# ElijahHyndman/PAPTeam_OpticalFlow

Measured on AMD Instinct MI355X. Metric: Mpix/s per frame-pair (fixed SOR iters) at 1920x1080; max-abs d(u,v) vs ref, higher is better.
Workload: dtype f64

## Files before the change

papteam_opticalflow_amd/csrc/sor.hip:

```cpp
#include <algorithm>
#include <cstdio>
#include <cstdlib>
#include <cstring>
#include <type_traits>

#include "common.h"

namespace papof {

namespace {

#ifndef PAPOF_V_DM6
#define PAPOF_V_DM6 4
#endif
#ifndef PAPOF_V_DM8
#define PAPOF_V_DM8 5
#endif
#ifndef PAPOF_V_FDM6
#define PAPOF_V_FDM6 3
#endif
#ifndef PAPOF_V_FDM8
#define PAPOF_V_FDM8 4
#endif
#ifndef PAPOF_V_FMIDPOLL
#define PAPOF_V_FMIDPOLL 10
#endif
#ifndef PAPOF_V_FSELECTIVE
#define PAPOF_V_FSELECTIVE false
#endif
#ifndef PAPOF_V_MIDPOLL
#define PAPOF_V_MIDPOLL 8
#endif
#ifndef PAPOF_V_SLEEP
#define PAPOF_V_SLEEP 1
#endif
constexpr int kProgStride = 32;
constexpr unsigned kSpinLimit = 4u << 20;

struct ExactArgs {
    const double *phi, *xy, *a1, *a2, *b1, *b2;
    double *du, *dv;
    unsigned* prog;
    unsigned* abort;
    int H, W, nb, ns, hp, npos, qt, rt, npos_d, n_sor;
    int xcd_affine;
    int k0;
    int b0, nbl;
    double nalpha, om1;
    unsigned long long* dbg;
    unsigned long long* stamp;
    double* peer_du;
    unsigned* peer_prog;
    int top_cut;
    int bot_cut;
    size_t bs_coef, bs_d, bs_prog;
    int skip_dead;
};

__device__ __forceinline__ void stamp_now(unsigned long long* s) {
    if (s && (blockIdx.x | threadIdx.x) == 0u) *s = __builtin_amdgcn_s_memrealtime();
}

__device__ __forceinline__ double ld_agent(const double* p) {
    return __hip_atomic_load(p, __ATOMIC_RELAXED, __HIP_MEMORY_SCOPE_AGENT);
}
__device__ __forceinline__ void st_agent(double* p, double v) {
    __hip_atomic_store(p, v, __ATOMIC_RELAXED, __HIP_MEMORY_SCOPE_AGENT);
}

template <bool DPP>
__device__ __forceinline__ double from_above(double x) {
    if (DPP) {
        int lo = __builtin_amdgcn_update_dpp(0, __double2loint(x), 0x138, 0xf, 0xf, true);
        int hi = __builtin_amdgcn_update_dpp(0, __double2hiint(x), 0x138, 0xf, 0xf, true);
        return __hiloint2double(hi, lo);
    }
    return __shfl_up(x, 1);
}
template <bool DPP>
__device__ __forceinline__ double from_below(double x) {
    if (DPP) {
        int lo = __builtin_amdgcn_update_dpp(0, __double2loint(x), 0x130, 0xf, 0xf, true);
        int hi = __builtin_amdgcn_update_dpp(0, __double2hiint(x), 0x130, 0xf, 0xf, true);
        return __hiloint2double(hi, lo);
    }
    return __shfl_down(x, 1);
}

__global__ void k_xlane_probe(int* out) {
    const int lane = threadIdx.x;
    const double v = (double)(lane + 1);
    out[lane] = (int)from_above<true>(v);
    out[64 + lane] = (int)from_below<true>(v);
}

typedef unsigned u32x4 __attribute__((ext_vector_type(4)));
struct D2 {
    double x, y;
};
__device__ __forceinline__ D2 as_d2(u32x4 v) {
    D2 r;
    __builtin_memcpy(&r, &v, sizeof r);
    return r;
}
__device__ __forceinline__ u32x4 as_u4(double x, double y) {
    D2 d{x, y};
    u32x4 r;
    __builtin_memcpy(&r, &d, sizeof r);
    return r;
}
constexpr int kAuxPlain = 0, kAuxSc1 = 16;
constexpr unsigned kOob = 0x80000000u;
constexpr unsigned kBlock = kLanes * 16u;

template <int T0, int T1, class F, class... Args>
__device__ __forceinline__ void static_for(F&& f, Args... args) {
    if constexpr (T0 < T1) {
        static_for<T0, T1 - 1>(f, args...);
        f(std::integral_constant<int, T1 - 1>{}, args...);
    }
}
template <int N, class F>
__device__ __forceinline__ void static_for(F&& f) {
    static_for<0, N>(f);
}

__device__ __forceinline__ D2 sor_cell(double wl, double duL, double dvL, double wu, double duU, double dvU, double wc,
                                       double duR, double dvR, double duD, double dvD, double nalpha, double xy,
                                       double duC, double dvC, double om1, double a1, double a2, double b1, double b2) {
    double s1 = wl * duL, s2 = wl * dvL;
    s1 += wc * duR;
    s2 += wc * dvR;
    s1 += wu * duU;
    s2 += wu * dvU;
    s1 += wc * duD;
    s2 += wc * dvD;
    s1 *= nalpha;
    s2 *= nalpha;
    s1 += xy * dvC;
    const double duN = om1 * duC + a1 * (b1 - s1);
    s2 += xy * duN;
    const double dvN = om1 * dvC + a2 * (b2 - s2);
    return D2{duN, dvN};
}

template <int R>
struct Slots {
    u32x4 pa[R], pb[R], pc[R];
    u32x4 pd[R];
};

struct Task {
    __amdgpu_buffer_rsrc_t ra, rb, rc, rd;
    __amdgpu_buffer_rsrc_t rp;
    __amdgpu_buffer_rsrc_t rd2, rp2;
};

__device__ __forceinline__ void publish(const Task& T, unsigned lane_off, unsigned steps) {
    __builtin_amdgcn_raw_buffer_store_b32(steps, T.rp, lane_off, 0, 16 );
}

struct BufAt {
    unsigned lane, uniform;
};
struct LaneOffs {
    unsigned pa;
    unsigned pbc;
    unsigned pd;
    unsigned st;
    unsigned pos_c;
    unsigned pos_d;
    unsigned hs;
    __device__ __forceinline__ BufAt unknowns_at(int s) const { return BufAt{pd, (unsigned)s * pos_d}; }
};

template <int R, int t, class Lane>
__device__ __forceinline__ void load_coef(const Task& T, const Lane& L, int s, Slots<R>& c) {
    const unsigned off = (unsigned)s * L.pos_c;
    c.pa[t] = __builtin_amdgcn_raw_buffer_load_b128(T.ra, L.pa, off, kAuxPlain);
    c.pb[t] = __builtin_amdgcn_raw_buffer_load_b128(T.rb, L.pbc, off, kAuxPlain);
    c.pc[t] = __builtin_amdgcn_raw_buffer_load_b128(T.rc, L.pbc, off, kAuxPlain);
}
template <int R, int t, class Lane>
__device__ __forceinline__ void load_unknowns(const Task& T, const Lane& L, int s, Slots<R>& c) {
    const BufAt at = L.unknowns_at(s);
    c.pd[t] = __builtin_amdgcn_raw_buffer_load_b128(T.rd, at.lane, at.uniform, kAuxSc1);
}
template <int R, int t, class Lane>
__device__ __forceinline__ void load_slot(const Task& T, const Lane& L, int s, Slots<R>& c) {
    load_coef<R, t>(T, L, s, c);
    load_unknowns<R, t>(T, L, s, c);
}
template <int R, class Lane>
__device__ __forceinline__ void fill_coef(const Task& T, const Lane& L, Slots<R>& c) {
    static_for<R>([&](auto t) __attribute__((always_inline)) { load_coef<R, t()>(T, L, t(), c); });
}
template <int R, class Lane>
__device__ __forceinline__ void fill_unknowns(const Task& T, const Lane& L, Slots<R>& c) {
    static_for<R>([&](auto t) __attribute__((always_inline)) { load_unknowns<R, t()>(T, L, t(), c); });
}

struct State {
    double duL, dvL, phiL, duC, dvC;
};

template <bool DPP>
__device__ __forceinline__ D2 wave_cell(const State& S, double om1, double nalpha, const D2& pa, const D2& pb,
                                        const D2& pc, double duR, double dvR) {
    const double duD = from_below<DPP>(duR);
    const double dvD = from_below<DPP>(dvR);
    const double leftU = S.phiL * S.duL;
    const double leftV = S.phiL * S.dvL;
    const double upU = from_above<DPP>(leftU);
    const double upV = from_above<DPP>(leftV);
    return sor_cell(1.0, leftU, leftV, 1.0, upU, upV, pa.x, duR, dvR, duD, dvD, nalpha, pa.y, S.duC, S.dvC, om1, pb.x, pb.y,
                    pc.x, pc.y);
}

__device__ __forceinline__ void store_data_guard() { asm volatile("s_nop 1" ::: "memory"); }

__device__ __forceinline__ double moved(double x) {
    double y;
    asm volatile("v_mov_b64 %0, %1" : "=v"(y) : "v"(x));
    return y;
}

template <int R, int t, bool DPP, bool SPLIT = false>
__device__ __forceinline__ void step(const ExactArgs& A, const Task& T, const LaneOffs& L, double om1, int s,
                                     Slots<R>& c, State& S) {
    const D2 pa = as_d2(c.pa[t]), pb = as_d2(c.pb[t]), pc = as_d2(c.pc[t]), pd = as_d2(c.pd[t]);
    const double phiC = pa.x, duR = pd.x, dvR = pd.y;
    const D2 n = wave_cell<DPP>(S, om1, A.nalpha, pa, pb, pc, duR, dvR);
    __builtin_amdgcn_raw_buffer_store_b128(as_u4(n.x, n.y), T.rd, L.st, (unsigned)s * L.pos_d, kAuxSc1);
    if (SPLIT)
        __builtin_amdgcn_raw_buffer_store_b128(as_u4(n.x, n.y), T.rd2, L.hs, (unsigned)s * L.pos_d, kAuxSc1);
    store_data_guard();
    S.duL = n.x;
    S.dvL = n.y;
    S.phiL = moved(phiC);
    S.duC = moved(duR);
    S.dvC = moved(dvR);
    asm volatile("" ::: "memory");
    load_slot<R, t>(T, L, s + R, c);
}

struct Polls {
    unsigned own, up, dn2;
};
struct Deps {
    unsigned *own, *up, *dn2;
    bool has_own, has_up, has_dn2;
};
__device__ __forceinline__ Polls poll(const Deps& d) {
    Polls p;
    p.own = d.has_own ? __hip_atomic_load(d.own, __ATOMIC_RELAXED, __HIP_MEMORY_SCOPE_AGENT) : 0x7fffffffu;
    p.up = d.has_up ? __hip_atomic_load(d.up, __ATOMIC_RELAXED, __HIP_MEMORY_SCOPE_AGENT) : 0x7fffffffu;
    p.dn2 = d.has_dn2 ? __hip_atomic_load(d.dn2, __ATOMIC_RELAXED, __HIP_MEMORY_SCOPE_AGENT) : 0x7fffffffu;
    return p;
}
__device__ __forceinline__ unsigned uni(unsigned v) { return (unsigned)__builtin_amdgcn_readfirstlane((int)v); }
__device__ __forceinline__ Polls uni(const Polls& p) { return Polls{uni(p.own), uni(p.up), uni(p.dn2)}; }

template <int OWN, int UP>
__device__ __forceinline__ bool covered(const Polls& p, int ns, int s_end) {
    return p.own >= (unsigned)min(ns, s_end + OWN) && p.up >= (unsigned)min(ns, s_end + UP) &&
           p.dn2 >= (unsigned)min(ns, max(0, s_end - 62));
}

__device__ __forceinline__ void end_task() { __builtin_amdgcn_endpgm(); }

template <int OWN, int UP, bool SELECTIVE = false>
__device__ __forceinline__ bool wait_covered(const ExactArgs& A, const Polls& pl, const Deps& d, int s_end) {
    Polls p = uni(pl);
    if (!covered<OWN, UP>(p, A.ns, s_end)) {
        unsigned spins = 0;
        do {
            __builtin_amdgcn_s_sleep(PAPOF_V_SLEEP);
            if ((++spins & 255u) == 0u) {
                if (uni(__hip_atomic_load(A.abort, __ATOMIC_RELAXED, __HIP_MEMORY_SCOPE_AGENT)) != 0u) return false;
                if (spins > kSpinLimit) {
                    __hip_atomic_store(A.abort, 1u, __ATOMIC_RELAXED, __HIP_MEMORY_SCOPE_AGENT);
                    return false;
                }
            }
            if (!SELECTIVE) {
                p = uni(poll(d));
                continue;
            }
            const unsigned need_own = (unsigned)min(A.ns, s_end + OWN), need_up = (unsigned)min(A.ns, s_end + UP);
            const unsigned need_dn2 = (unsigned)min(A.ns, max(0, s_end - 62));
            if (p.own < need_own) p.own = uni(__hip_atomic_load(d.own, __ATOMIC_RELAXED, __HIP_MEMORY_SCOPE_AGENT));
            if (p.up < need_up) p.up = uni(__hip_atomic_load(d.up, __ATOMIC_RELAXED, __HIP_MEMORY_SCOPE_AGENT));
            if (p.dn2 < need_dn2) p.dn2 = uni(__hip_atomic_load(d.dn2, __ATOMIC_RELAXED, __HIP_MEMORY_SCOPE_AGENT));
        } while (!covered<OWN, UP>(p, A.ns, s_end));
    }
    __builtin_amdgcn_fence(__ATOMIC_ACQUIRE, "wavefront");
    return true;
}

__device__ __forceinline__ bool task_of_block(const ExactArgs& A, int& u, int& b) {
    if (A.xcd_affine) {
        const int nf = A.nb >> 3, rem = A.nb & 7, S = 8 * nf + (rem ? 8 : 0);
        const int ul = blockIdx.x / S;
        u = A.k0 + ul;
        const int r = blockIdx.x - ul * S;
        if (r < 8 * nf) {
            b = r;
        } else {
            const int j = r - 8 * nf - (nf ? u % (9 - rem) : 0);
            b = 8 * nf + j;
            if (j < 0 || j >= rem) return false;
        }
    } else {
        const int ul = blockIdx.x / A.nbl;
        u = A.k0 + ul;
        b = A.b0 + (blockIdx.x - ul * A.nbl);
    }
    return true;
}

__device__ __forceinline__ unsigned plane_descriptors(const ExactArgs& A, Task& T) {
    const unsigned plane_bytes = (unsigned)(((size_t)A.npos * A.hp + kLanes) * 16u);
    const unsigned par_bytes = (unsigned)A.npos_d * (unsigned)A.nb * kBlock;
    T.ra = __builtin_amdgcn_make_buffer_rsrc((void*)A.phi, 0, plane_bytes, 0x00020000);
    T.rb = __builtin_amdgcn_make_buffer_rsrc((void*)A.a1, 0, plane_bytes, 0x00020000);
    T.rc = __builtin_amdgcn_make_buffer_rsrc((void*)A.b1, 0, plane_bytes, 0x00020000);
    T.rd = __builtin_amdgcn_make_buffer_rsrc((void*)A.du, 0, 2u * par_bytes, 0x00020000);
    return par_bytes;
}

struct Pipe {
    Polls pl;
    unsigned ma, mb;
};
template <int R, int DM, bool MIDPOLL, int OWN, int UP, bool SELECTIVE, class Run, class Publish>
__device__ __forceinline__ void pipeline_iteration(const ExactArgs& A, const Deps& D, const State& S, Pipe& P, int i,
                                                   bool first, Run&& run, Publish&& publish) {
    constexpr int H = R / 2;
    constexpr int CA = H + DM - R, CB = DM;
    static_assert(CA >= 0 && CA < H && CB >= H && CB < R, "marker consumption points");
    if (!wait_covered<OWN, UP, SELECTIVE>(A, P.pl, D, (i + 2) * R)) end_task();
    Polls pn{0u, 0u, 0u};
    if (!MIDPOLL) pn = poll(D);
    static_for<0, CA>(run, i * R);
    if (!first) {
        asm volatile("" ::"v"(P.ma), "v"(S.duL), "v"(S.dvL) : "memory");
        if (uni(P.ma) != 0u) end_task();
        publish((unsigned)min(A.ns, (i - 1) * R + H));
    }
    static_for<CA, H>(run, i * R);
    P.ma = __hip_atomic_load(A.abort, __ATOMIC_RELAXED, __HIP_MEMORY_SCOPE_AGENT);
    if (MIDPOLL) pn = poll(D);
    static_for<H, CB>(run, i * R);
    if (!first) {
        asm volatile("" ::"v"(P.mb), "v"(S.duL), "v"(S.dvL) : "memory");
        if (uni(P.mb) != 0u) end_task();
        publish((unsigned)min(A.ns, i * R));
    }
    static_for<CB, R>(run, i * R);
    P.mb = __hip_atomic_load(A.abort, __ATOMIC_RELAXED, __HIP_MEMORY_SCOPE_AGENT);
    P.pl = pn;
}

template <int R, bool DPP, bool SPLIT = false>
__global__ __launch_bounds__(64) void k_sor_exact(ExactArgs A_in) {
    static_assert(R >= 4 && R % 2 == 0, "two markers per iteration");
    ExactArgs A = A_in;
    {
        const size_t p = blockIdx.y;
        A.phi += p * A.bs_coef;
        A.a1 += p * A.bs_coef;
        A.b1 += p * A.bs_coef;
        A.du += p * A.bs_d;
        A.prog += p * A.bs_prog;
    }
    stamp_now(A.stamp);
    const unsigned lane = threadIdx.x;
    int k, b;
    if (!task_of_block(A, k, b)) return;
    const int ns = A.ns;
    const bool ghost = lane == 0 || lane == kLanes - 1;
    unsigned long long* const dbg = A.dbg ? A.dbg + (size_t)(k * A.nb + b) * 8 : nullptr;
    if (dbg) dbg[0] = __builtin_amdgcn_s_memrealtime();
    Task T;
    const unsigned par_bytes = plane_descriptors(A, T);
    const int r0 = kBandRows * b - k - 1;
    LaneOffs L;
    L.pos_c = (unsigned)A.hp * 16u;
    L.pos_d = (unsigned)A.nb * kBlock;
    const unsigned base = ((unsigned)(r0 + A.qt) * (unsigned)A.hp + (unsigned)(r0 + A.rt) + lane) * 16u;
    const int row = r0 + (int)lane;
    const bool dead = !SPLIT && A.skip_dead != 0 && (row < 0 || row >= A.H);
    L.pa = dead ? kOob : base;
    L.pbc = (ghost || dead) ? kOob : base;
    const unsigned mine = (unsigned)(k & 1) * par_bytes, prev = (unsigned)((k + 1) & 1) * par_bytes;
    L.st = dead ? kOob : mine + L.pos_d + (unsigned)b * kBlock + lane * 16u;
    const bool cut_top = SPLIT && A.top_cut && b == A.b0, cut_bot = SPLIT && A.bot_cut && b == A.b0 + A.nbl - 1;
    const unsigned up_cell = cut_top ? (unsigned)(k >> 1) : 62u;
    const unsigned pd_above = b > 0 ? mine + 64u * L.pos_d + (unsigned)(b - 1) * kBlock + up_cell * 16u : kOob;
    L.hs = (cut_bot && lane == kLanes - 2) ? mine + L.pos_d + (unsigned)b * kBlock + (unsigned)(k >> 1) * 16u : kOob;
    T.rd2 = __builtin_amdgcn_make_buffer_rsrc((void*)((SPLIT && A.peer_du) ? A.peer_du : A.du), 0, 2u * par_bytes, 0x00020000);
    L.pd = dead ? kOob : (lane == 0 ? pd_above : (k > 0 ? prev + L.pos_d + (unsigned)b * kBlock + (lane - 1u) * 16u : kOob));
    const double om1 = ghost ? 1.0 : A.om1;

    const unsigned prog_bytes = (unsigned)A.n_sor * (unsigned)A.nb * kProgStride * 4u;
    T.rp = __builtin_amdgcn_make_buffer_rsrc((void*)A.prog, 0, prog_bytes, 0x00020000);
    T.rp2 = __builtin_amdgcn_make_buffer_rsrc((void*)((SPLIT && A.peer_prog) ? A.peer_prog : A.prog), 0, prog_bytes, 0x00020000);
    const unsigned my_prog = lane == 0 ? (unsigned)(k * A.nb + b) * kProgStride * 4u : kOob;
    const unsigned my_prog2 = cut_bot ? my_prog : kOob;
    Deps D;
    D.has_own = k > 0;
    D.has_up = b > 0;
    D.has_dn2 = k > 1 && b + 1 < A.nb && !cut_bot;
    D.own = A.prog + ((size_t)(k - 1) * A.nb + b) * kProgStride;
    D.up = A.prog + ((size_t)k * A.nb + (b - 1)) * kProgStride;
    D.dn2 = A.prog + ((size_t)(k - 2) * A.nb + (b + 1)) * kProgStride;
    const auto publish_all = [&](unsigned steps) {
        publish(T, my_prog, steps);
        if (SPLIT) __builtin_amdgcn_raw_buffer_store_b32(steps, T.rp2, my_prog2, 0, 16 );
    };

    const int n_iter = (ns + R - 1) / R;
    State S;
    S.duL = S.dvL = S.phiL = 0.0;
    Slots<R> c;

    fill_coef(T, L, c);
    Pipe P{poll(D), 0u, 0u};
    if (!wait_covered<0, 63, true>(A, P.pl, D, R)) end_task();
    {
        const unsigned first = (lane != 0 || L.pd == kOob) ? kOob : L.pd - L.pos_d;
        const D2 c0 = as_d2(__builtin_amdgcn_raw_buffer_load_b128(T.rd, first, 0, kAuxSc1));
        S.duC = c0.x;
        S.dvC = c0.y;
    }
    if (dbg) dbg[1] = __builtin_amdgcn_s_memrealtime();
    fill_unknowns(T, L, c);
    P.pl = poll(D);

    constexpr int DM = R >= 10 ? R - 3 : (R == 8 ? PAPOF_V_DM8 : (R == 6 ? PAPOF_V_DM6 : R / 2));
    const auto iteration = [&](int i, bool first) {
        pipeline_iteration<R, DM, R >= PAPOF_V_MIDPOLL, 0, 63, true>(
            A, D, S, P, i, first,
            [&](auto t, int s0) __attribute__((always_inline)) { step<R, t(), DPP, SPLIT>(A, T, L, om1, s0 + t(), c, S); },
            publish_all);
    };
    iteration(0, true);
    if (dbg) dbg[2] = __builtin_amdgcn_s_memrealtime();
    for (int i = 1; i < n_iter; ++i) {
        iteration(i, false);
        if (dbg && i < 4) dbg[2 + i] = __builtin_amdgcn_s_memrealtime();
    }
    asm volatile("s_waitcnt vmcnt(0)" ::: "memory");
    publish_all((unsigned)ns);
    if (dbg) dbg[6] = __builtin_amdgcn_s_memrealtime();
}

struct FLane {
    unsigned m1;
    double om1a;
    double om1b;
    bool first_out;
    bool own_block;
};

template <int R, int t, bool DPP, bool SKIP2, bool ID2>
__device__ __forceinline__ void f_step(const ExactArgs& A, const Task& T, const LaneOffs& L, const FLane& F, int s,
                                       Slots<R>& c, State& S1, State& S2) {
    const double nalpha = A.nalpha;
    constexpr int t2 = (t + R - 2) % R;
    const double duR2 = S1.duL, dvR2 = S1.dvL;
    double duN2, dvN2;
    if (SKIP2) {
        duN2 = 0.0;
        dvN2 = 0.0;
    } else {
        const D2 qa = as_d2(c.pa[t2]), qc = as_d2(c.pc[t2]);
        const u32x4 qbm = ID2 ? (c.pb[t2] & u32x4{0u, 0u, 0u, 0u}) : c.pb[t2];
        const D2 qb = as_d2(qbm);
        const D2 n2 = wave_cell<DPP>(S2, F.om1b, nalpha, qa, qb, qc, duR2, dvR2);
        duN2 = n2.x;
        dvN2 = n2.y;
        S2.phiL = moved(qa.x);
    }
    const D2 pa = as_d2(c.pa[t]), pc = as_d2(c.pc[t]), pd = as_d2(c.pd[t]);
    const u32x4 pbm = c.pb[t] & u32x4{F.m1, F.m1, F.m1, F.m1};
    const D2 pb = as_d2(pbm);
    const double phiC = pa.x, duR = pd.x, dvR = pd.y;
    const D2 n1 = wave_cell<DPP>(S1, F.om1a, nalpha, pa, pb, pc, duR, dvR);
    const double duN = n1.x, dvN = n1.y;
    const double o1 = F.first_out ? duN : duN2, o2 = F.first_out ? dvN : dvN2;
    __builtin_amdgcn_raw_buffer_store_b128(as_u4(o1, o2), T.rd, L.st, (unsigned)s * L.pos_d, kAuxSc1);
    store_data_guard();
    S2.duL = duN2;
    S2.dvL = dvN2;
    S2.duC = duR2;
    S2.dvC = dvR2;
    S1.duL = duN;
    S1.dvL = dvN;
    S1.phiL = phiC;
    S1.duC = moved(duR);
    S1.dvC = moved(dvR);
    asm volatile("" ::: "memory");
    load_unknowns<R, t>(T, L, s + R, c);
    if (!SKIP2) load_coef<R, t2>(T, L, s - 2 + R, c);
}

template <int R, bool DPP, bool ID2>
__device__ __forceinline__ void f_run(const ExactArgs& A, const Task& T, const LaneOffs& L, const FLane& F,
                                      const Deps& D, unsigned my_prog) {
    const int ns = A.ns;
    const int n_iter = (ns + R - 1) / R;
    State S1, S2;
    S1.duL = S1.dvL = S1.phiL = 0.0;
    S2.duL = S2.dvL = S2.phiL = S2.duC = S2.dvC = 0.0;
    Slots<R> c;
    fill_coef(T, L, c);
    Pipe P{poll(D), 0u, 0u};
    if (!wait_covered<1, 64, PAPOF_V_FSELECTIVE>(A, P.pl, D, R)) end_task();
    {
        const unsigned first = (F.own_block || L.pd == kOob) ? kOob : L.pd - L.pos_d;
        const D2 c0 = as_d2(__builtin_amdgcn_raw_buffer_load_b128(T.rd, first, 0, kAuxSc1));
        S1.duC = c0.x;
        S1.dvC = c0.y;
    }
    fill_unknowns(T, L, c);
    P.pl = poll(D);
    constexpr int DM = R == 6 ? PAPOF_V_FDM6 : (R == 8 ? PAPOF_V_FDM8 : R - 3);
    const auto iteration = [&](int i, auto first) {
        pipeline_iteration<R, DM, R >= PAPOF_V_FMIDPOLL, 1, 64, PAPOF_V_FSELECTIVE>(
            A, D, S1, P, i, first(),
            [&](auto t, int s0) __attribute__((always_inline)) {
                f_step<R, t(), DPP, first() && t() < 2, ID2>(A, T, L, F, s0 + t(), c, S1, S2);
            },
            [&](unsigned steps) __attribute__((always_inline)) { publish(T, my_prog, steps); });
    };
    iteration(0, std::true_type{});
    for (int i = 1; i < n_iter; ++i) iteration(i, std::false_type{});
    asm volatile("s_waitcnt vmcnt(0)" ::: "memory");
    publish(T, my_prog, (unsigned)ns);
}

template <int R, bool DPP>
__global__ __launch_bounds__(64) void k_sor_fused(ExactArgs A) {
    static_assert(R >= 6 && R % 2 == 0, "two markers per iteration; coefficient slots live two extra steps");
    stamp_now(A.stamp);
    const unsigned lane = threadIdx.x;
    const int pairs = (A.n_sor + 1) >> 1;
    int q, b;
    if (!task_of_block(A, q, b)) return;
    Task T;
    const unsigned par_bytes = plane_descriptors(A, T);
    const int r0 = kFusedRows * b - 2 * q - 2;
    LaneOffs L;
    L.pos_c = (unsigned)A.hp * 16u;
    L.pos_d = (unsigned)A.nb * kBlock;
    const unsigned base = ((unsigned)(r0 + A.qt) * (unsigned)A.hp + (unsigned)(r0 + A.rt) + lane) * 16u;
    L.pa = base;
    L.pbc = (lane == 0 || lane == kLanes - 1) ? kOob : base;
    const unsigned mine = (unsigned)(q & 1) * par_bytes, prev = (unsigned)((q + 1) & 1) * par_bytes;
    L.st = lane == kLanes - 1 ? kOob : mine + L.pos_d + (unsigned)b * kBlock + lane * 16u;
    const unsigned pd1 = b > 0 ? mine + 63u * L.pos_d + (unsigned)(b - 1) * kBlock + 62u * 16u : kOob;
    const unsigned pd0 = b > 0 ? mine + 65u * L.pos_d + (unsigned)(b - 1) * kBlock + 61u * 16u : kOob;
    const unsigned pd_own = q > 0 ? prev + 2u * L.pos_d + (unsigned)b * kBlock + (lane - 2u) * 16u : kOob;
    L.pd = lane == 0 ? pd0 : (lane == 1 ? pd1 : pd_own);
    FLane F;
    const bool real1 = lane >= 2 && lane <= kLanes - 2;
    F.m1 = real1 ? 0xffffffffu : 0u;
    F.om1a = real1 ? A.om1 : 1.0;
    F.om1b = (lane == 0 || lane == kLanes - 1) ? 1.0 : A.om1;
    if ((A.n_sor & 1) && q == pairs - 1) F.om1b = 1.0;
    F.first_out = lane == kLanes - 2;
    F.own_block = lane >= 2;

    const unsigned prog_bytes = (unsigned)A.n_sor * (unsigned)A.nb * kProgStride * 4u;
    T.rp = __builtin_amdgcn_make_buffer_rsrc((void*)A.prog, 0, prog_bytes, 0x00020000);
    const unsigned my_prog = lane == 0 ? (unsigned)(q * A.nb + b) * kProgStride * 4u : kOob;
    Deps D;
    D.has_own = q > 0;
    D.has_up = b > 0;
    D.has_dn2 = q > 1 && b + 1 < A.nb;
    D.own = A.prog + ((size_t)(q - 1) * A.nb + b) * kProgStride;
    D.up = A.prog + ((size_t)q * A.nb + (b - 1)) * kProgStride;
    D.dn2 = A.prog + ((size_t)(q - 2) * A.nb + (b + 1)) * kProgStride;
    if ((A.n_sor & 1) && q == pairs - 1)
        f_run<R, DPP, true>(A, T, L, F, D, my_prog);
    else
        f_run<R, DPP, false>(A, T, L, F, D, my_prog);
}

struct GroupArgs {
    const double *phi, *a1, *b1;
    double* du;
    unsigned* prog;
    unsigned* abort;
    int nb, ns, hp, npos, qt, rt, npos_d, n_sor;
    int xcd_affine;
    int g0;
    unsigned long long* dbg;
    unsigned halo_off;
    double nalpha, om1;
    unsigned long long* stamp;
};

constexpr int kRing = 16;

struct GLane {
    unsigned pa, pbc;
    unsigned pd, pd_step;
    unsigned st;
    unsigned hs;
    unsigned pos_c, pos_d;
    __device__ __forceinline__ BufAt unknowns_at(int s) const { return BufAt{pd + (unsigned)s * pd_step, 0u}; }
};

typedef __attribute__((address_space(3))) u32x4 lds_u32x4;
typedef __attribute__((address_space(3))) volatile unsigned lds_word;

template <int R, int t, bool DPP, bool FROM_LDS, bool TO_LDS>
__device__ __forceinline__ void g_step(const GroupArgs& A, const Task& T, const GLane& L, lds_u32x4* ring_out,
                                       unsigned lane, double om1, int s, Slots<R>& c, const u32x4 (&lpd)[R / 2],
                                       State& S) {
    const D2 pa = as_d2(c.pa[t]), pb = as_d2(c.pb[t]), pc = as_d2(c.pc[t]);
    u32x4 raw = c.pd[t];
    if (FROM_LDS) {
        const u32x4 l = lpd[t % (R / 2)];
        raw = lane != 0 ? l : raw;
    }
    const D2 pd = as_d2(raw);
    const double phiC = pa.x, duR = pd.x, dvR = pd.y;
    const D2 n = wave_cell<DPP>(S, om1, A.nalpha, pa, pb, pc, duR, dvR);
    const u32x4 out = as_u4(n.x, n.y);
    if (TO_LDS)
        ring_out[(s & (kRing - 1)) * kLanes + lane] = out;
    else
        __builtin_amdgcn_raw_buffer_store_b128(out, T.rd, L.st, (unsigned)s * L.pos_d, kAuxSc1);
    __builtin_amdgcn_raw_buffer_store_b128(out, T.rd, L.hs + (unsigned)s * 16u, 0, kAuxSc1);
    store_data_guard();
    S.duL = n.x;
    S.dvL = n.y;
    S.phiL = moved(phiC);
    S.duC = moved(duR);
    S.dvC = moved(dvR);
    asm volatile("" ::: "memory");
    load_slot<R, t>(T, L, s + R, c);
}

template <int R, int T0, int T1, bool DPP, bool FROM_LDS, bool TO_LDS>
__device__ __forceinline__ void g_steps(const GroupArgs& A, const Task& T, const GLane& L, lds_u32x4* ring_out,
                                        unsigned lane, double om1, int s0, Slots<R>& c, const u32x4 (&lpd)[R / 2],
                                        State& S) {
    static_for<T0, T1>([&](auto t) __attribute__((always_inline)) {
        g_step<R, t(), DPP, FROM_LDS, TO_LDS>(A, T, L, ring_out, lane, om1, s0 + t(), c, lpd, S);
    });
}

__device__ __forceinline__ void lds_store_lane0(lds_word* p, unsigned v) {
    unsigned long long saved;
    asm volatile("s_mov_b64 %0, exec\n\ts_mov_b64 exec, 1\n\tds_write_b32 %1, %2\n\ts_mov_b64 exec, %0"
                 : "=&s"(saved)
                 : "v"((unsigned)(unsigned long long)(const volatile void __attribute__((address_space(3)))*)p), "v"(v)
                 : "memory");
}
__device__ __forceinline__ bool lds_wait_ge(lds_word* p, unsigned need, lds_word* group_abort) {
    unsigned spins = 0;
    while (uni(*p) < need) {
        __builtin_amdgcn_s_sleep(1);
        if ((++spins & 255u) == 0u && (uni(*group_abort) != 0u || spins > (kSpinLimit << 3))) return false;
    }
    asm volatile("" ::: "memory");
    return true;
}

struct GWaveCtx {
    lds_u32x4 *ring_in, *ring_out;
    lds_word *done_in, *taken_in, *done_out, *taken_out;
    lds_word* group_abort;
    int task;
    unsigned my_prog;
    Deps D;
    int ns, n_iter;
};

template <int R, bool DPP, bool FROM_LDS, bool TO_LDS>
__device__ __forceinline__ void g_run_wave(const GroupArgs& A, const Task& T, const GLane& L, const GWaveCtx& W,
                                           unsigned lane, double om1) {
    constexpr int H = R / 2;
    const int ns = W.ns;
    ExactArgs X;
    X.abort = A.abort;
    X.ns = ns;
    const auto give_up = [&]() {
        lds_store_lane0(W.group_abort, 1u);
        __hip_atomic_store(A.abort, 1u, __ATOMIC_RELAXED, __HIP_MEMORY_SCOPE_AGENT);
    };
    State S;
    S.duL = S.dvL = S.phiL = 0.0;
    Slots<R> c;
    u32x4 lpd[H];
#pragma unroll
    for (int q = 0; q < H; q++) lpd[q] = u32x4{0u, 0u, 0u, 0u};
    const unsigned lcell = lane > 0 ? lane - 1u : 0u;

    unsigned long long t_cov = 0, t_in = 0, t_out = 0, t_start = 0;
    const bool dbg = A.dbg != nullptr;
    fill_coef(T, L, c);
    Polls pl = poll(W.D);
    if (!wait_covered<1, 63>(X, pl, W.D, 2 * R)) return give_up();
    if (dbg) t_start = __builtin_amdgcn_s_memtime();
    {
        const unsigned first = L.pd == kOob ? kOob : L.pd - L.pd_step;
        const D2 c0 = as_d2(__builtin_amdgcn_raw_buffer_load_b128(T.rd, first, 0, kAuxSc1));
        S.duC = c0.x;
        S.dvC = c0.y;
    }
    fill_unknowns(T, L, c);

    const auto half_begin = [&](int sa) -> bool {
        if (FROM_LDS) {
            const unsigned long long ta = dbg ? __builtin_amdgcn_s_memtime() : 0;
            if (!lds_wait_ge(W.done_in, (unsigned)(sa + H), W.group_abort)) return false;
            if (dbg) t_in += __builtin_amdgcn_s_memtime() - ta;
#pragma unroll
            for (int q = 0; q < H; q++) lpd[q] = W.ring_in[((sa + q) & (kRing - 1)) * kLanes + lcell];
        }
        const unsigned long long tb = dbg ? __builtin_amdgcn_s_memtime() : 0;
        if (TO_LDS && sa + H > kRing && !lds_wait_ge(W.taken_out, (unsigned)(sa + H - kRing), W.group_abort))
            return false;
        if (dbg) t_out += __builtin_amdgcn_s_memtime() - tb;
        return true;
    };
    const auto half_end = [&](int sa) {
        if (FROM_LDS) {
            asm volatile("" ::: "memory");
            lds_store_lane0(W.taken_in, (unsigned)(sa + H));
        }
        if (TO_LDS) {
            asm volatile("s_waitcnt lgkmcnt(0)" ::: "memory");
            lds_store_lane0(W.done_out, (unsigned)(sa + H));
        }
    };

    constexpr int DL = R - 3, CA = H + DL - R, CB = DL;
    static_assert(CA >= 0 && CA < H && CB >= H && CB < R, "marker consumption points");
    unsigned ma = 0u, mb = 0u;
    const auto iteration = [&](int i, bool first) -> bool {
        const unsigned long long tc = dbg ? __builtin_amdgcn_s_memtime() : 0;
        if (!first && !wait_covered<1, 63>(X, pl, W.D, (i + 2) * R)) return false;
        if (dbg) t_cov += __builtin_amdgcn_s_memtime() - tc;
        const Polls pn = poll(W.D);
        const int s0 = i * R;
        if (!half_begin(s0)) return false;
        g_steps<R, 0, CA, DPP, FROM_LDS, TO_LDS>(A, T, L, W.ring_out, lane, om1, s0, c, lpd, S);
        if (!first) {
            asm volatile("" ::"v"(ma), "v"(S.duL), "v"(S.dvL) : "memory");
            if (uni(ma) != 0u) return false;
            publish(T, W.my_prog, (unsigned)min(ns, s0 - R + H));
        }
        g_steps<R, CA, H, DPP, FROM_LDS, TO_LDS>(A, T, L, W.ring_out, lane, om1, s0, c, lpd, S);
        ma = __hip_atomic_load(A.abort, __ATOMIC_RELAXED, __HIP_MEMORY_SCOPE_AGENT);
        half_end(s0);
        if (!half_begin(s0 + H)) return false;
        g_steps<R, H, CB, DPP, FROM_LDS, TO_LDS>(A, T, L, W.ring_out, lane, om1, s0, c, lpd, S);
        if (!first) {
            asm volatile("" ::"v"(mb), "v"(S.duL), "v"(S.dvL) : "memory");
            if (uni(mb) != 0u) return false;
            publish(T, W.my_prog, (unsigned)min(ns, s0));
        }
        g_steps<R, CB, R, DPP, FROM_LDS, TO_LDS>(A, T, L, W.ring_out, lane, om1, s0, c, lpd, S);
        mb = __hip_atomic_load(A.abort, __ATOMIC_RELAXED, __HIP_MEMORY_SCOPE_AGENT);
        half_end(s0 + H);
        pl = pn;
        return true;
    };
    if (!iteration(0, true)) return give_up();
    for (int i = 1; i < W.n_iter; ++i)
        if (!iteration(i, false)) return give_up();
    asm volatile("s_waitcnt vmcnt(0)" ::: "memory");
    publish(T, W.my_prog, (unsigned)ns);
    if (dbg) {
        unsigned long long* o = A.dbg + (size_t)W.task * 4;
        o[0] = __builtin_amdgcn_s_memtime() - t_start;
        o[1] = t_cov;
        o[2] = t_in;
        o[3] = t_out;
    }
}

template <int R, int M, bool DPP>
__global__ __launch_bounds__(64 * M) void k_sor_group(GroupArgs A) {
    static_assert(R >= 6 && R % 2 == 0 && R <= kRing, "half-iterations of R/2 steps; the ring holds two of them");
    __shared__ u32x4 ring[(M > 1 ? M - 1 : 1) * kRing * kLanes];
    __shared__ unsigned lds_done[M];
    __shared__ unsigned lds_taken[M];
    __shared__ unsigned lds_abort;
    stamp_now(A.stamp);
    const unsigned lane = threadIdx.x & 63u;
    const int m = __builtin_amdgcn_readfirstlane((int)(threadIdx.x >> 6));
    lds_store_lane0((lds_word*)&lds_done[m], 0u);
    lds_store_lane0((lds_word*)&lds_taken[m], 0u);
    lds_store_lane0((lds_word*)&lds_abort, 0u);
    __syncthreads();
    int g, b;
    if (A.xcd_affine) {
        const int x = blockIdx.x & 7, y = blockIdx.x >> 3, nb8 = (A.nb + 7) >> 3;
        const int gl = y / nb8;
        g = A.g0 + gl;
        b = (y - gl * nb8) * 8 + x;
        if (b >= A.nb) return;
    } else {
        const int gl = blockIdx.x / A.nb;
        g = A.g0 + gl;
        b = blockIdx.x - gl * A.nb;
    }
    const int k = g * M + m;
    if (k >= A.n_sor) return;
    const bool ghost = lane == 0 || lane == kLanes - 1;
    const bool from_lds = m > 0, to_planes = m == M - 1 || k == A.n_sor - 1;
    GWaveCtx W;
    lds_u32x4* const ring3 = (lds_u32x4*)ring;
    W.ring_in = ring3 + (m > 0 ? m - 1 : 0) * kRing * kLanes;
    W.ring_out = ring3 + (m < M - 1 ? m : 0) * kRing * kLanes;
    W.done_in = (lds_word*)&lds_done[m > 0 ? m - 1 : 0];
    W.taken_in = (lds_word*)&lds_taken[m > 0 ? m - 1 : 0];
    W.done_out = (lds_word*)&lds_done[m];
    W.taken_out = (lds_word*)&lds_taken[m];
    W.group_abort = (lds_word*)&lds_abort;
    W.task = k * A.nb + b;
    W.ns = A.ns;
    W.n_iter = (A.ns + R - 1) / R;

    Task T;
    const unsigned plane_bytes = (unsigned)(((size_t)A.npos * A.hp + kLanes) * 16u);
    const unsigned par_bytes = (unsigned)A.npos_d * (unsigned)A.nb * kBlock;
    const unsigned all_bytes = A.halo_off + (unsigned)A.n_sor * (unsigned)A.nb * (unsigned)A.npos_d * 16u;
    T.ra = __builtin_amdgcn_make_buffer_rsrc((void*)A.phi, 0, plane_bytes, 0x00020000);
    T.rb = __builtin_amdgcn_make_buffer_rsrc((void*)A.a1, 0, plane_bytes, 0x00020000);
    T.rc = __builtin_amdgcn_make_buffer_rsrc((void*)A.b1, 0, plane_bytes, 0x00020000);
    T.rd = __builtin_amdgcn_make_buffer_rsrc((void*)A.du, 0, all_bytes, 0x00020000);
    const int r0 = kBandRows * b - k - 1;
    GLane L;
    L.pos_c = (unsigned)A.hp * 16u;
    L.pos_d = (unsigned)A.nb * kBlock;
    const unsigned base = ((unsigned)(r0 + A.qt) * (unsigned)A.hp + (unsigned)(r0 + A.rt) + lane) * 16u;
    L.pa = base;
    L.pbc = ghost ? kOob : base;
    const unsigned mine = (unsigned)(g & 1) * par_bytes, prev = (unsigned)((g + 1) & 1) * par_bytes;
    L.st = to_planes ? mine + L.pos_d + (unsigned)b * kBlock + lane * 16u : kOob;
    const auto halo_row = [&](int kk, int bb) {
        return A.halo_off + (unsigned)((kk * A.nb + bb) * A.npos_d) * 16u;
    };
    const unsigned pd_halo = b > 0 ? halo_row(k, b - 1) + 64u * 16u : kOob;
    const unsigned pd_plane = prev + L.pos_d + (unsigned)b * kBlock + (lane - 1u) * 16u;
    L.pd = lane == 0 ? pd_halo : (from_lds ? kOob : pd_plane);
    L.pd_step = lane == 0 ? 16u : (from_lds ? 0u : L.pos_d);
    L.hs = (lane == kLanes - 2 && b + 1 < A.nb) ? halo_row(k, b) + 16u : kOob;
    const double om1 = ghost ? 1.0 : A.om1;

    T.rp = __builtin_amdgcn_make_buffer_rsrc((void*)A.prog, 0, (unsigned)A.n_sor * (unsigned)A.nb * kProgStride * 4u, 0x00020000);
    W.my_prog = lane == 0 ? (unsigned)(k * A.nb + b) * kProgStride * 4u : kOob;
    W.D.has_own = m == 0 && k > 0;
    W.D.has_up = b > 0;
    W.D.has_dn2 = false;
    W.D.own = A.prog + ((size_t)(k - 1) * A.nb + b) * kProgStride;
    W.D.up = A.prog + ((size_t)k * A.nb + (b - 1)) * kProgStride;
    W.D.dn2 = W.D.own;
    if (from_lds) {
        if (to_planes)
            g_run_wave<R, DPP, true, false>(A, T, L, W, lane, om1);
        else
            g_run_wave<R, DPP, true, true>(A, T, L, W, lane, om1);
    } else {
        if (to_planes)
            g_run_wave<R, DPP, false, false>(A, T, L, W, lane, om1);
        else
            g_run_wave<R, DPP, false, true>(A, T, L, W, lane, om1);
    }
}

typedef double f64x2 __attribute__((ext_vector_type(2)));

struct BlockedArgs {
    const double *phi, *xy, *a1, *a2, *b1, *b2;
    const double *su, *sv;
    double *du, *dv;
    int H, W;
    Rect out;
    int g;
    int hs0;
    int cw, ch, ntx, nblk;
    int shift;
    unsigned long long* stamp;
    double nalpha, om1;
};

template <bool VEC>
__device__ __forceinline__ f64x2 load_pair(const double* __restrict__ plane, size_t o, bool ok0, bool ok1) {
    f64x2 r = {0.0, 0.0};
    if (VEC) {
        if (ok0) r = *reinterpret_cast<const f64x2*>(plane + o);
    } else {
        if (ok0) r.x = plane[o];
        if (ok1) r.y = plane[o + 1];
    }
    return r;
}

template <int MODE, int NW, int RPT, bool VEC>
__global__ __launch_bounds__(NW * 64) void k_sor_blocked(BlockedArgs A) {
    constexpr int RH = NW * RPT, S = kLanes + 1, CELLS = (RH + 2) * S + 2;
    __shared__ f64x2 lds[2][CELLS];
    stamp_now(A.stamp);
    const int t = threadIdx.x & 63;
    const int w = __builtin_amdgcn_readfirstlane((int)(threadIdx.x >> 6));
    const int per = (A.nblk + 7) >> 3;
    const int tile = (int)(blockIdx.x & 7u) * per + (int)(blockIdx.x >> 3);
    if ((int)(blockIdx.x >> 3) >= per || tile >= A.nblk) return;
    const int by = tile / A.ntx, bx = tile - by * A.ntx;
    const int cx0 = A.out.x0 + bx * A.cw, cx1 = min(cx0 + A.cw, A.out.x1);
    const int cy0 = A.out.y0 + by * A.ch, cy1 = min(cy0 + A.ch, A.out.y1);
    const int rx0 = max(0, cx0 - A.g - A.shift), rx1 = min(A.W, cx1 + A.g);
    const int ry0 = max(0, cy0 - A.g), ry1 = min(A.H, cy1 + A.g);
    const int W = A.W;
    const int j0 = rx0 + 2 * t;
    const int r0 = w * RPT;
    const int q0 = (ry0 + rx0 + r0) & 1;

    double ph[RPT][3], up[2], cxy[RPT][2], ca1[RPT][2], ca2[RPT][2], cb1[RPT][2], cb2[RPT][2];
    f64x2 u0[RPT], v0[RPT];
    {
        const int iu = ry0 + r0 - 1;
        const bool rok = iu >= 0 && iu < ry1;
        const f64x2 pu = load_pair<VEC>(A.phi, (size_t)max(iu, 0) * W + j0, rok && j0 < rx1, rok && j0 + 1 < rx1);
        up[0] = pu.x;
        up[1] = pu.y;
    }
    static_for<RPT>([&](auto RR) __attribute__((always_inline)) {
        constexpr int rr = decltype(RR)::value;
        const int i = ry0 + r0 + rr;
        const bool rok = i < ry1, ok0 = rok && j0 < rx1, ok1 = rok && j0 + 1 < rx1;
        const size_t o = (size_t)min(i, A.H - 1) * W + j0;
        const f64x2 p = load_pair<VEC>(A.phi, o, ok0, ok1);
        const f64x2 x = load_pair<VEC>(A.xy, o, ok0, ok1);
        const f64x2 q1 = load_pair<VEC>(A.a1, o, ok0, ok1);
        const f64x2 q2 = load_pair<VEC>(A.a2, o, ok0, ok1);
        const f64x2 e1 = load_pair<VEC>(A.b1, o, ok0, ok1);
        const f64x2 e2 = load_pair<VEC>(A.b2, o, ok0, ok1);
        u0[rr] = f64x2{0.0, 0.0};
        v0[rr] = f64x2{0.0, 0.0};
        if (A.su) {
            u0[rr] = load_pair<VEC>(A.su, o, ok0, ok1);
            v0[rr] = load_pair<VEC>(A.sv, o, ok0, ok1);
        }
        ph[rr][1] = p.x;
        ph[rr][2] = p.y;
        cxy[rr][0] = x.x;
        cxy[rr][1] = x.y;
        ca1[rr][0] = q1.x;
        ca1[rr][1] = q1.y;
        ca2[rr][0] = q2.x;
        ca2[rr][1] = q2.y;
        cb1[rr][0] = e1.x;
        cb1[rr][1] = e1.y;
        cb2[rr][0] = e2.x;
        cb2[rr][1] = e2.y;
    });
    static_for<RPT>([&](auto RR) __attribute__((always_inline)) {
        constexpr int rr = decltype(RR)::value;
        const double left = __shfl_up(ph[rr][2], 1);
        ph[rr][0] = t == 0 ? 0.0 : left;
    });

    const int idx0 = (r0 + 1) * S + t + 1;
    static_for<RPT>([&](auto RR) __attribute__((always_inline)) {
        constexpr int rr = decltype(RR)::value;
        const int c0 = (q0 + rr) & 1;
        lds[c0][idx0 + rr * S] = f64x2{u0[rr].x, v0[rr].x};
        lds[c0 ^ 1][idx0 + rr * S] = f64x2{u0[rr].y, v0[rr].y};
        if (t == 0) {
            lds[0][idx0 + rr * S - 1] = f64x2{0.0, 0.0};
            lds[1][idx0 + rr * S - 1] = f64x2{0.0, 0.0};
        }
    });
    if (w == 0) {
        lds[0][t] = f64x2{0.0, 0.0};
        lds[1][t] = f64x2{0.0, 0.0};
        if (t == 0) {
            lds[0][S - 1] = f64x2{0.0, 0.0};
            lds[1][S - 1] = f64x2{0.0, 0.0};
        }
    }
    if (w == NW - 1) {
        lds[0][(RH + 1) * S + t] = f64x2{0.0, 0.0};
        lds[1][(RH + 1) * S + t] = f64x2{0.0, 0.0};
        if (t < 3) {
            lds[0][(RH + 1) * S + 64 + t - 1 + 1] = f64x2{0.0, 0.0};
            lds[1][(RH + 1) * S + 64 + t - 1 + 1] = f64x2{0.0, 0.0};
        }
    }
    __syncthreads();

    const int ox0 = rx0 > 0, ox1 = rx1 < A.W, oy0 = ry0 > 0, oy1 = ry1 < A.H;
    const int rw = rx1 - rx0, rh = ry1 - ry0;
    const double nalpha = A.nalpha, om1 = A.om1;
    const auto cell = [&](auto RR, auto PP, int cc) __attribute__((always_inline)) -> f64x2 {
        constexpr int rr = decltype(RR)::value, p = decltype(PP)::value;
        const int idx = idx0 + rr * S;
        const f64x2* __restrict__ Lo = lds[cc ^ 1];
        const f64x2 own = lds[cc][idx];
        const f64x2 L = Lo[idx - 1 + p], R = Lo[idx + p], U = Lo[idx - S], D = Lo[idx + S];
        const double pc = ph[rr][1 + p], wl = ph[rr][p];
        double wu;
        if constexpr (rr > 0)
            wu = ph[rr - 1][1 + p];
        else
            wu = up[p];
        const D2 n = sor_cell(wl, L.x, L.y, wu, U.x, U.y, pc, R.x, R.y, D.x, D.y, nalpha, cxy[rr][p], own.x,
                              own.y, om1, ca1[rr][p], ca2[rr][p], cb1[rr][p], cb2[rr][p]);
        return f64x2{n.x, n.y};
    };
    if (MODE == PAPOF_SOR_REDBLACK) {
        const auto half = [&](auto PARC, int m, int c) __attribute__((always_inline)) {
            constexpr int PAR = decltype(PARC)::value;
            const int fx0 = ox0 * (m + 1), fx1 = rw - ox1 * (m + 1), fy0 = oy0 * (m + 1), fy1 = rh - oy1 * (m + 1);
            if (r0 + RPT <= fy0 || r0 >= fy1) {
                __syncthreads();
                return;
            }
            if constexpr (NW < 16) {
                constexpr int IL = NW == 12 ? 2 : RPT;
                static_assert(RPT % IL == 0, "row groups");
                static_for<RPT / IL>([&](auto GG) __attribute__((always_inline)) {
                    constexpr int g0 = decltype(GG)::value * IL;
                    f64x2 nw[IL];
                    static_for<IL>([&](auto QQ) __attribute__((always_inline)) {
                        constexpr int rr = g0 + decltype(QQ)::value;
                        nw[decltype(QQ)::value] = cell(std::integral_constant<int, rr>{}, std::integral_constant<int, (PAR + rr) & 1>{}, c);
                    });
                    static_for<IL>([&](auto QQ) __attribute__((always_inline)) {
                        constexpr int rr = g0 + decltype(QQ)::value;
                        constexpr int p = (PAR + rr) & 1;
                        const int r = r0 + rr, lc = 2 * t + p;
                        if (r >= fy0 && r < fy1 && lc >= fx0 && lc < fx1) lds[c][idx0 + rr * S] = nw[decltype(QQ)::value];
                    });
                });
            } else {
                static_for<RPT>([&](auto RR) __attribute__((always_inline)) {
                    constexpr int rr = decltype(RR)::value;
                    constexpr int p = (PAR + rr) & 1;
                    const int r = r0 + rr;
                    if (r >= fy0 && r < fy1) {
// ... 880 lines not shown
```

Before: 213.8.

## Shorten unknowns prefetch lead by one step and split phi from a/b loads

Changes the software pipeline in the wavefront SOR kernels so the unknowns (du,dv) and phi slots are refilled one step later (R-1 ahead) while a/b coefficients stay R ahead. The dependency wait thresholds drop by one step, so waves can start an iteration sooner after upstream progress. It also removes the explicit v_mov_b64 register copies by tying the store-data hazard guard to the stored values. The risk is less latency hiding for the unknown loads and subtle slot-indexing or hazard mistakes.

```diff
diff --git a/papteam_opticalflow_amd/csrc/sor.hip b/papteam_opticalflow_amd/csrc/sor.hip
--- a/papteam_opticalflow_amd/csrc/sor.hip
+++ b/papteam_opticalflow_amd/csrc/sor.hip
@@ -171,13 +171,21 @@
     unsigned pos_c;
     unsigned pos_d;
     unsigned hs;
-    __device__ __forceinline__ BufAt unknowns_at(int s) const { return BufAt{pd, (unsigned)s * pos_d}; }
+    int pd_lead = 0;
+    __device__ __forceinline__ void lead_unknowns(int steps) {
+        pd = pd == kOob ? kOob : pd + (unsigned)steps * pos_d;
+        pd_lead = steps;
+    }
+    __device__ __forceinline__ BufAt unknowns_at(int s) const { return BufAt{pd, (unsigned)(s - pd_lead) * pos_d}; }
 };
 
 template <int R, int t, class Lane>
-__device__ __forceinline__ void load_coef(const Task& T, const Lane& L, int s, Slots<R>& c) {
+__device__ __forceinline__ void load_phi(const Task& T, const Lane& L, int s, Slots<R>& c) {
+    c.pa[t] = __builtin_amdgcn_raw_buffer_load_b128(T.ra, L.pa, (unsigned)s * L.pos_c, kAuxPlain);
+}
+template <int R, int t, class Lane>
+__device__ __forceinline__ void load_ab(const Task& T, const Lane& L, int s, Slots<R>& c) {
     const unsigned off = (unsigned)s * L.pos_c;
-    c.pa[t] = __builtin_amdgcn_raw_buffer_load_b128(T.ra, L.pa, off, kAuxPlain);
     c.pb[t] = __builtin_amdgcn_raw_buffer_load_b128(T.rb, L.pbc, off, kAuxPlain);
     c.pc[t] = __builtin_amdgcn_raw_buffer_load_b128(T.rc, L.pbc, off, kAuxPlain);
 }
@@ -187,17 +195,26 @@
     c.pd[t] = __builtin_amdgcn_raw_buffer_load_b128(T.rd, at.lane, at.uniform, kAuxSc1);
 }
 template <int R, int t, class Lane>
-__device__ __forceinline__ void load_slot(const Task& T, const Lane& L, int s, Slots<R>& c) {
-    load_coef<R, t>(T, L, s, c);
-    load_unknowns<R, t>(T, L, s, c);
-}
-template <int R, class Lane>
+__device__ __forceinline__ void refill(const Task& T, const Lane& L, int s, Slots<R>& c) {
+    constexpr int tp = (t + R - 1) % R;
+    load_phi<R, tp>(T, L, s + R - 1, c);
+    load_ab<R, t>(T, L, s + R, c);
+    load_unknowns<R, tp>(T, L, s + R - 1, c);
+}
+template <int R>
+__device__ __forceinline__ constexpr int unknowns_end(int i) {
+    return (i + 2) * R - 1;
+}
+template <int R, int NPHI, class Lane>
 __device__ __forceinline__ void fill_coef(const Task& T, const Lane& L, Slots<R>& c) {
-    static_for<R>([&](auto t) __attribute__((always_inline)) { load_coef<R, t()>(T, L, t(), c); });
+    static_for<R>([&](auto t) __attribute__((always_inline)) {
+        if constexpr (t() < NPHI) load_phi<R, t()>(T, L, t(), c);
+        load_ab<R, t()>(T, L, t(), c);
+    });
 }
 template <int R, class Lane>
 __device__ __forceinline__ void fill_unknowns(const Task& T, const Lane& L, Slots<R>& c) {
-    static_for<R>([&](auto t) __attribute__((always_inline)) { load_unknowns<R, t()>(T, L, t(), c); });
+    static_for<R - 1>([&](auto t) __attribute__((always_inline)) { load_unknowns<R, t()>(T, L, t(), c); });
 }
 
 struct State {
@@ -218,11 +235,12 @@
 }
 
 __device__ __forceinline__ void store_data_guard() { asm volatile("s_nop 1" ::: "memory"); }
-
-__device__ __forceinline__ double moved(double x) {
-    double y;
-    asm volatile("v_mov_b64 %0, %1" : "=v"(y) : "v"(x));
-    return y;
+__device__ __forceinline__ D2 store_data_guard(u32x4 data) {
+    asm volatile("s_nop 1" : "+v"(data) : : "memory");
+    return as_d2(data);
+}
+__device__ __forceinline__ void store_data_guard(const u32x4& data, double& x, double& y) {
+    asm volatile("s_nop 1" : "+v"(x), "+v"(y) : "v"(data) : "memory");
 }
 
 template <int R, int t, bool DPP, bool SPLIT = false>
@@ -231,17 +249,18 @@
     const D2 pa = as_d2(c.pa[t]), pb = as_d2(c.pb[t]), pc = as_d2(c.pc[t]), pd = as_d2(c.pd[t]);
     const double phiC = pa.x, duR = pd.x, dvR = pd.y;
     const D2 n = wave_cell<DPP>(S, om1, A.nalpha, pa, pb, pc, duR, dvR);
-    __builtin_amdgcn_raw_buffer_store_b128(as_u4(n.x, n.y), T.rd, L.st, (unsigned)s * L.pos_d, kAuxSc1);
+    const u32x4 out = as_u4(n.x, n.y);
+    __builtin_amdgcn_raw_buffer_store_b128(out, T.rd, L.st, (unsigned)s * L.pos_d, kAuxSc1);
     if (SPLIT)
-        __builtin_amdgcn_raw_buffer_store_b128(as_u4(n.x, n.y), T.rd2, L.hs, (unsigned)s * L.pos_d, kAuxSc1);
-    store_data_guard();
-    S.duL = n.x;
-    S.dvL = n.y;
-    S.phiL = moved(phiC);
-    S.duC = moved(duR);
-    S.dvC = moved(dvR);
+        __builtin_amdgcn_raw_buffer_store_b128(out, T.rd2, L.hs, (unsigned)s * L.pos_d, kAuxSc1);
+    const D2 left = store_data_guard(out);
+    S.duL = left.x;
+    S.dvL = left.y;
+    S.phiL = phiC;
+    S.duC = duR;
+    S.dvC = dvR;
     asm volatile("" ::: "memory");
-    load_slot<R, t>(T, L, s + R, c);
+    refill<R, t>(T, L, s, c);
 }
 
 struct Polls {
@@ -339,7 +358,7 @@
     constexpr int H = R / 2;
     constexpr int CA = H + DM - R, CB = DM;
     static_assert(CA >= 0 && CA < H && CB >= H && CB < R, "marker consumption points");
-    if (!wait_covered<OWN, UP, SELECTIVE>(A, P.pl, D, (i + 2) * R)) end_task();
+    if (!wait_covered<OWN, UP, SELECTIVE>(A, P.pl, D, unknowns_end<R>(i))) end_task();
     Polls pn{0u, 0u, 0u};
     if (!MIDPOLL) pn = poll(D);
     static_for<0, CA>(run, i * R);
@@ -425,9 +444,9 @@
     S.duL = S.dvL = S.phiL = 0.0;
     Slots<R> c;
 
-    fill_coef(T, L, c);
+    fill_coef<R, R - 1>(T, L, c);
     Pipe P{poll(D), 0u, 0u};
-    if (!wait_covered<0, 63, true>(A, P.pl, D, R)) end_task();
+    if (!wait_covered<0, 63, true>(A, P.pl, D, unknowns_end<R>(-1))) end_task();
     {
         const unsigned first = (lane != 0 || L.pd == kOob) ? kOob : L.pd - L.pos_d;
         const D2 c0 = as_d2(__builtin_amdgcn_raw_buffer_load_b128(T.rd, first, 0, kAuxSc1));
@@ -436,6 +455,7 @@
     }
     if (dbg) dbg[1] = __builtin_amdgcn_s_memrealtime();
     fill_unknowns(T, L, c);
+    L.lead_unknowns(R - 1);
     P.pl = poll(D);
 
     constexpr int DM = R >= 10 ? R - 3 : (R == 8 ? PAPOF_V_DM8 : (R == 6 ? PAPOF_V_DM6 : R / 2));
@@ -464,11 +484,14 @@
     bool own_block;
 };
 
-template <int R, int t, bool DPP, bool SKIP2, bool ID2>
+template <int R, int t, bool DPP, int EARLY, bool ID2>
 __device__ __forceinline__ void f_step(const ExactArgs& A, const Task& T, const LaneOffs& L, const FLane& F, int s,
                                        Slots<R>& c, State& S1, State& S2) {
     const double nalpha = A.nalpha;
+    constexpr bool SKIP2 = EARLY < 2;
     constexpr int t2 = (t + R - 2) % R;
+    constexpr int t3 = (t + R - 3) % R;
+    constexpr int tp = (t + R - 1) % R;
     const double duR2 = S1.duL, dvR2 = S1.dvL;
     double duN2, dvN2;
     if (SKIP2) {
@@ -481,7 +504,7 @@
         const D2 n2 = wave_cell<DPP>(S2, F.om1b, nalpha, qa, qb, qc, duR2, dvR2);
         duN2 = n2.x;
         dvN2 = n2.y;
-        S2.phiL = moved(qa.x);
+        S2.phiL = qa.x;
     }
     const D2 pa = as_d2(c.pa[t]), pc = as_d2(c.pc[t]), pd = as_d2(c.pd[t]);
     const u32x4 pbm = c.pb[t] & u32x4{F.m1, F.m1, F.m1, F.m1};
@@ -490,24 +513,26 @@
     const D2 n1 = wave_cell<DPP>(S1, F.om1a, nalpha, pa, pb, pc, duR, dvR);
     const double duN = n1.x, dvN = n1.y;
     const double o1 = F.first_out ? duN : duN2, o2 = F.first_out ? dvN : dvN2;
-    __builtin_amdgcn_raw_buffer_store_b128(as_u4(o1, o2), T.rd, L.st, (unsigned)s * L.pos_d, kAuxSc1);
-    store_data_guard();
+    const u32x4 out = as_u4(o1, o2);
+    __builtin_amdgcn_raw_buffer_store_b128(out, T.rd, L.st, (unsigned)s * L.pos_d, kAuxSc1);
     S2.duL = duN2;
     S2.dvL = dvN2;
     S2.duC = duR2;
     S2.dvC = dvR2;
     S1.duL = duN;
     S1.dvL = dvN;
+    store_data_guard(out, S1.duL, S1.dvL);
     S1.phiL = phiC;
-    S1.duC = moved(duR);
-    S1.dvC = moved(dvR);
+    S1.duC = duR;
+    S1.dvC = dvR;
     asm volatile("" ::: "memory");
-    load_unknowns<R, t>(T, L, s + R, c);
-    if (!SKIP2) load_coef<R, t2>(T, L, s - 2 + R, c);
+    load_unknowns<R, tp>(T, L, s + R - 1, c);
+    if (EARLY >= 3) load_phi<R, t3>(T, L, s - 3 + R, c);
+    if (!SKIP2) load_ab<R, t2>(T, L, s - 2 + R, c);
 }
 
 template <int R, bool DPP, bool ID2>
-__device__ __forceinline__ void f_run(const ExactArgs& A, const Task& T, const LaneOffs& L, const FLane& F,
+__device__ __forceinline__ void f_run(const ExactArgs& A, const Task& T, LaneOffs L, const FLane& F,
                                       const Deps& D, unsigned my_prog) {
     const int ns = A.ns;
     const int n_iter = (ns + R - 1) / R;
@@ -515,9 +540,9 @@
     S1.duL = S1.dvL = S1.phiL = 0.0;
     S2.duL = S2.dvL = S2.phiL = S2.duC = S2.dvC = 0.0;
     Slots<R> c;
-    fill_coef(T, L, c);
+    fill_coef<R, R>(T, L, c);
     Pipe P{poll(D), 0u, 0u};
-    if (!wait_covered<1, 64, PAPOF_V_FSELECTIVE>(A, P.pl, D, R)) end_task();
+    if (!wait_covered<1, 64, PAPOF_V_FSELECTIVE>(A, P.pl, D, unknowns_end<R>(-1))) end_task();
     {
         const unsigned first = (F.own_block || L.pd == kOob) ? kOob : L.pd - L.pos_d;
         const D2 c0 = as_d2(__builtin_amdgcn_raw_buffer_load_b128(T.rd, first, 0, kAuxSc1));
@@ -525,13 +550,14 @@
         S1.dvC = c0.y;
     }
     fill_unknowns(T, L, c);
+    L.lead_unknowns(R - 1);
     P.pl = poll(D);
     constexpr int DM = R == 6 ? PAPOF_V_FDM6 : (R == 8 ? PAPOF_V_FDM8 : R - 3);
     const auto iteration = [&](int i, auto first) {
         pipeline_iteration<R, DM, R >= PAPOF_V_FMIDPOLL, 1, 64, PAPOF_V_FSELECTIVE>(
             A, D, S1, P, i, first(),
             [&](auto t, int s0) __attribute__((always_inline)) {
-                f_step<R, t(), DPP, first() && t() < 2, ID2>(A, T, L, F, s0 + t(), c, S1, S2);
+                f_step<R, t(), DPP, (first() && t() < 3) ? t() : 3, ID2>(A, T, L, F, s0 + t(), c, S1, S2);
             },
             [&](unsigned steps) __attribute__((always_inline)) { publish(T, my_prog, steps); });
     };
@@ -636,14 +662,14 @@
     else
         __builtin_amdgcn_raw_buffer_store_b128(out, T.rd, L.st, (unsigned)s * L.pos_d, kAuxSc1);
     __builtin_amdgcn_raw_buffer_store_b128(out, T.rd, L.hs + (unsigned)s * 16u, 0, kAuxSc1);
-    store_data_guard();
-    S.duL = n.x;
-    S.dvL = n.y;
-    S.phiL = moved(phiC);
-    S.duC = moved(duR);
-    S.dvC = moved(dvR);
+    const D2 left = store_data_guard(out);
+    S.duL = left.x;
+    S.dvL = left.y;
+    S.phiL = phiC;
+    S.duC = duR;
+    S.dvC = dvR;
     asm volatile("" ::: "memory");
-    load_slot<R, t>(T, L, s + R, c);
+    refill<R, t>(T, L, s, c);
 }
 
 template <int R, int T0, int T1, bool DPP, bool FROM_LDS, bool TO_LDS>
@@ -704,9 +730,9 @@
 
     unsigned long long t_cov = 0, t_in = 0, t_out = 0, t_start = 0;
     const bool dbg = A.dbg != nullptr;
-    fill_coef(T, L, c);
+    fill_coef<R, R - 1>(T, L, c);
     Polls pl = poll(W.D);
-    if (!wait_covered<1, 63>(X, pl, W.D, 2 * R)) return give_up();
+    if (!wait_covered<1, 63>(X, pl, W.D, unknowns_end<R>(0))) return give_up();
     if (dbg) t_start = __builtin_amdgcn_s_memtime();
     {
         const unsigned first = L.pd == kOob ? kOob : L.pd - L.pd_step;
@@ -746,7 +772,7 @@
     unsigned ma = 0u, mb = 0u;
     const auto iteration = [&](int i, bool first) -> bool {
         const unsigned long long tc = dbg ? __builtin_amdgcn_s_memtime() : 0;
-        if (!first && !wait_covered<1, 63>(X, pl, W.D, (i + 2) * R)) return false;
+        if (!first && !wait_covered<1, 63>(X, pl, W.D, unknowns_end<R>(i))) return false;
         if (dbg) t_cov += __builtin_amdgcn_s_memtime() - tc;
         const Polls pn = poll(W.D);
         const int s0 = i * R;
```

New measurement: 216.2 (median of 6 runs). +1.1%, better.
